# SpursLipu/YOLOv3v4-ModelCompression-MultidatasetTraining-Multibackbone

Measured on AMD Instinct MI355X. Metric: images/sec YOLOv3-608 train fp16, higher is better.
Workload: dtype f16; 1 GPU; YOLOv3 Darknet-53 608 COCO (80 classes) fp16 training step, batch 64/GPU: train-mode forward (batch-stat BN) + compute_loss + backward + nesterov SGD, single GPU; global_batch=64, parallelism=dp1

## Files before the change

yolov3v4-modelcompression-multidatasettraining-multibackbone_amd/csrc/conv_igemm.hip:

```cpp
#include "conv_igemm.h"

namespace yh {

template <typename T, int TM, int TN, int KU> struct MmaStep;

template <int TM, int TN, int KU> struct MmaStep<f16, TM, TN, KU> {
    static __device__ __forceinline__ void run(const u32x4* As, const u32x4* Bs, int BM, int BN, int arow, int brow,
                                               int lane, f32x4 (&acc)[TM][TN]) {
        const int r = lane & 15;
#pragma unroll
        for (int h = 0; h < KU / 4; ++h) {
            const int u = h * 4 + (lane >> 4);
            f16x8 a[TM], b[TN];
#pragma unroll
            for (int i = 0; i < TM; ++i) {
                u32x4 v = As[u * BM + arow + i * 16 + r];
                a[i] = *reinterpret_cast<f16x8*>(&v);
            }
#pragma unroll
            for (int j = 0; j < TN; ++j) {
                u32x4 v = Bs[u * BN + brow + j * 16 + r];
                b[j] = *reinterpret_cast<f16x8*>(&v);
            }
#pragma unroll
// ... 248 lines not shown
        for (int i = 0; i < TM; ++i)
#pragma unroll
            for (int j = 0; j < TN; ++j)
                acc[i][j] = __builtin_amdgcn_mfma_f32_16x16x32_f16(a[i], b[j], acc[i][j], 0, 0, 0);
    }
};
template <int TM, int TN> struct MmaStepRM<float, TM, TN> {
    static __device__ __forceinline__ void run(const u32x4* As, const u32x4* Bs, int arow, int brow, int lane,
                                               f32x4 (&acc)[TM][TN]) {
        const int r = lane & 15, kq = lane >> 4, fr = swz_f(r >> 2);
        const float* Af = reinterpret_cast<const float*>(As);
        const float* Bf = reinterpret_cast<const float*>(Bs);
#pragma unroll
        for (int u = 0; u < 4; ++u) {
            const int off = (r * 4 + (u ^ fr)) * 4 + kq;
            float a[TM], b[TN];
#pragma unroll
            for (int i = 0; i < TM; ++i) a[i] = Af[(arow + i * 16) * 16 + off];
#pragma unroll
            for (int j = 0; j < TN; ++j) b[j] = Bf[(brow + j * 16) * 16 + off];
#pragma unroll
            for (int i = 0; i < TM; ++i)
#pragma unroll
                for (int j = 0; j < TN; ++j)
                    acc[i][j] = __builtin_amdgcn_mfma_f32_16x16x4f32(a[i], b[j], acc[i][j], 0, 0, 0);
        }
    }
};

template <int TM, int TN> struct MmaStepRM<int8_t, TM, TN> {
    static __device__ __forceinline__ void run(const u32x4* As, const u32x4* Bs, int arow, int brow, int lane,
                                               i32x4 (&acc)[TM][TN]) {
        const int r = lane & 15;
        const int off = r * 4 + ((lane >> 4) ^ swz_f(r >> 2));
        i32x4 a[TM], b[TN];
#pragma unroll
        for (int i = 0; i < TM; ++i) {
            u32x4 v = As[(arow + i * 16) * 4 + off];
            a[i] = *reinterpret_cast<i32x4*>(&v);
        }
#pragma unroll
        for (int j = 0; j < TN; ++j) {
            u32x4 v = Bs[(brow + j * 16) * 4 + off];
            b[j] = *reinterpret_cast<i32x4*>(&v);
        }
#pragma unroll
        for (int i = 0; i < TM; ++i)
#pragma unroll
            for (int j = 0; j < TN; ++j)
                acc[i][j] = __builtin_amdgcn_mfma_i32_16x16x64_i8(a[i], b[j], acc[i][j], 0, 0, 0);
    }
};

template <typename T, typename OutT, int BM, int BN, int WM, int WN, int STAGES, int ABL = 0>
__global__ __launch_bounds__(WM * WN * 64, (WM * WN * 2) / 4) void conv_igemm_glds_kernel(const ConvArgs a) {
    constexpr int VEC = Prec<T>::VEC, BK = VEC * 4;
    constexpr int NW = WM * WN;
    constexpr int TM = BM / WM / 16, TN = BN / WN / 16;
    constexpr int GA = BM / 16, GB = BN / 16;
    constexpr int GPW = (GA + GB) / NW;
    constexpr int GAW = GA / NW;
    static_assert(GA % NW == 0 && GB % NW == 0, "tile rows must split evenly over the waves");
    static_assert(STAGES == 3 || STAGES == 4, "3 or 4 stage ring");

    __shared__ u32x4 smem[STAGES * 4 * (BM + BN)];
    constexpr int STAGE_CELLS = 4 * (BM + BN);

    const int lane = threadIdx.x & 63;
    const int wave = __builtin_amdgcn_readfirstlane(threadIdx.x >> 6);
    const int wm = wave / WN, wn = wave % WN;

    int m_tile, p_tile;
    {
        const int nb = gridDim.x, bid = blockIdx.x;
        const int q = nb >> 3, rr = nb & 7, xcd = bid & 7;
        const int logical = (xcd < rr ? xcd * (q + 1) : rr * (q + 1) + (xcd - rr) * q) + (bid >> 3);
        p_tile = logical / a.m_tiles;
        m_tile = logical - p_tile * a.m_tiles;
    }
    const int m0 = m_tile * BM;
    const long p0 = (long)p_tile * BN;

    const int lrow = lane >> 2;
    const int lu = (lane & 3) ^ swz_f(lane >> 4);
    const T* const xg = reinterpret_cast<const T*>(a.x);
    const T* const zero = reinterpret_cast<const T*>(g_zero_page);

    const T* wsrc[GAW > 0 ? GAW : 1];
    static_for<GAW>([&](auto c) {
        constexpr int i = decltype(c)::value;
        const int row = min(m0 + (wave + i * NW) * 16 + lrow, a.m_pad - 1);
        wsrc[i] = reinterpret_cast<const T*>(a.w) + (long)row * a.ktot + lu * VEC;
    });
    constexpr int GBW = GPW - GAW;
    long bbase[GBW];
    int bhi[GBW], bwi[GBW];
    const int HoWo = a.Ho * a.Wo;
    static_for<GBW>([&](auto c) {
        constexpr int i = decltype(c)::value;
        const int row = (wave + i * NW) * 16 + lrow;
        const long p = p0 + row;
        if (p < a.P) {
            const int n = (int)(p / HoWo);
            const int rem = (int)(p - (long)n * HoWo);
            const int ho = rem / a.Wo, wo = rem - ho * a.Wo;
            bhi[i] = ho * a.stride - a.pad;
            bwi[i] = wo * a.stride - a.pad;
            bbase[i] = (((long)n * a.H + bhi[i]) * a.W + bwi[i]) * a.ldx + lu * VEC;
        } else {
            bhi[i] = -(1 << 28);
            bwi[i] = -(1 << 28);
            bbase[i] = 0;
        }
    });

    int kr = 0, ks = 0, kc = 0, kofs = 0;
    auto issue = [&](int st) {
        u32x4* const base = smem + st * STAGE_CELLS;
        if constexpr (ABL != 1) static_for<GAW>([&](auto c) {
            constexpr int i = decltype(c)::value;
            u32x4* dst = base + (wave + i * NW) * 64;
            __builtin_amdgcn_global_load_lds((const __attribute__((address_space(1))) void*)(wsrc[i] + kofs),
                                             (__attribute__((address_space(3))) void*)dst, 16, 0, 0);
        });
        const long tap = ((long)kr * a.W + ks) * a.ldx + kc;
        const bool cok = kc + lu * VEC < a.Cin;
        if constexpr (ABL != 1) static_for<GBW>([&](auto c) {
            constexpr int i = decltype(c)::value;
            const bool ok = cok && (unsigned)(bhi[i] + kr) < (unsigned)a.H && (unsigned)(bwi[i] + ks) < (unsigned)a.W;
            const T* src = ok ? xg + bbase[i] + tap : zero;
            u32x4* dst = base + 4 * BM + (wave + i * NW) * 64;
            __builtin_amdgcn_global_load_lds((const __attribute__((address_space(1))) void*)src,
                                             (__attribute__((address_space(3))) void*)dst, 16, 0, 0);
        });
        kofs += BK;
        kc += BK;
        if (kc >= a.cin_k) {
            kc = 0;
            if (++ks == a.S) { ks = 0; ++kr; }
        }
    };

    typedef typename AccOf<T>::type acc_t;
    acc_t acc[TM][TN];
#pragma unroll
    for (int i = 0; i < TM; ++i)
#pragma unroll
        for (int j = 0; j < TN; ++j) acc[i][j] = acc_t{0, 0, 0, 0};

    const int nk = a.ktot / BK;
#pragma unroll
    for (int s = 0; s < STAGES - 1; ++s)
        if (s < nk) issue(s);
    int st_read = 0, st_write = STAGES - 1;
    for (int kt = 0; kt < nk; ++kt) {
        const int ahead = min(STAGES - 2, nk - 1 - kt);
        if (ahead >= 2) wait_vmcnt<2 * GPW>();
        else if (ahead == 1) wait_vmcnt<GPW>();
        else wait_vmcnt<0>();
        __builtin_amdgcn_s_barrier();
        if (kt + STAGES - 1 < nk) issue(st_write);
        const u32x4* As = smem + st_read * STAGE_CELLS;
        if constexpr (ABL != 2) MmaStepRM<T, TM, TN>::run(As, As + 4 * BM, wm * TM * 16, wn * TN * 16, lane, acc);
        st_read = st_read + 1 == STAGES ? 0 : st_read + 1;
        st_write = st_write + 1 == STAGES ? 0 : st_write + 1;
    }

    conv_epilogue<T, OutT, TM, TN, BN, WN>(a, acc, m0, p0, wm, wn, lane);
}

template <typename T, typename OutT, int BM, int BN, int WM, int WN, int STAGES, int ABL = 0>
static int launch_glds(const ConvArgs& a0, hipStream_t stream) {
    ConvArgs a = a0;
    a.m_tiles = (a.Cout + BM - 1) / BM;
    a.p_tiles = (int)((a.P + BN - 1) / BN);
    const long blocks = (long)a.m_tiles * a.p_tiles;
    if (blocks <= 0 || blocks > 0x7fffffffL) return YH_EINVAL;
    hipLaunchKernelGGL((conv_igemm_glds_kernel<T, OutT, BM, BN, WM, WN, STAGES, ABL>), dim3((unsigned)blocks),
                       dim3(WM * WN * 64), 0, stream, a);
    return check_launch();
}


template <typename T, typename OutT, int BM, int LB>
__global__ __launch_bounds__(512, (BM <= 128 ? 4 : 2)) void conv3x3_halo_kernel(const ConvArgs a, const int rows_h) {
    constexpr int VEC = Prec<T>::VEC, BK = VEC * 4, BN = 256, NW = 8, WN = 4, STAGES = 3;
    constexpr int WM = NW / WN;
    constexpr int TM = BM / WM / 16, TN = BN / WN / 16;
    constexpr int GAW = BM / 16 / NW;
    static_assert(BM % (16 * NW) == 0, "weight tile must split over 8 waves");
    constexpr int LA = GAW;

    extern __shared__ __attribute__((aligned(16))) u32x4 dsm[];
    u32x4* const Aring = dsm;
    u32x4* const Bbuf0 = dsm + STAGES * BM * 4;
    u32x4* const dummy = Bbuf0 + 2 * rows_h * 4;

    const int lane = threadIdx.x & 63;
    const int wave = __builtin_amdgcn_readfirstlane(threadIdx.x >> 6);
    const int wm = wave / WN, wn = wave % WN;

    int m_tile, p_tile;
    {
        const int nb = gridDim.x, bid = blockIdx.x;
        const int q = nb >> 3, rr = nb & 7, xcd = bid & 7;
        const int logical = (xcd < rr ? xcd * (q + 1) : rr * (q + 1) + (xcd - rr) * q) + (bid >> 3);
        p_tile = logical / a.m_tiles;
        m_tile = logical - p_tile * a.m_tiles;
    }
    const int m0 = m_tile * BM;
    const long q0 = (long)p_tile * BN;
    const int Wp = a.W + 2;
    const long IMG = (long)(a.H + 1) * Wp;

    const int lrow = lane >> 2;
    const int lu = (lane & 3) ^ (((lane >> 4) & 1) << 1);
    const T* const xg = reinterpret_cast<const T*>(a.x);
    const T* const zero = reinterpret_cast<const T*>(g_zero_page);

    const T* wsrc[GAW];
    static_for<GAW>([&](auto c) {
        constexpr int i = decltype(c)::value;
        const int row = min(m0 + (wave + i * NW) * 16 + lrow, a.m_pad - 1);
        wsrc[i] = reinterpret_cast<const T*>(a.w) + (long)row * a.ktot + lu * VEC;
    });
    const long v0 = q0 - Wp - 1;
    const T* bsrc[LB];
    static_for<LB>([&](auto c) {
        constexpr int i = decltype(c)::value;
        const int j = (wave + i * NW) * 16 + lrow;
        const long v = v0 + j;
// ... 363 lines not shown
    size_t lds;
    if (!yh::hpp_geometry(d->w_in, d->cin_k, bk, &rows_hp, &lb, &hbufs, &lds)) return false;
    if ((long)d->n * d->h * d->w_in * d->ldx + d->cin_k >= 0x7fffffffL || (long)d->m_pad * 9 * d->cin_k >= 0x7fffffffL) return false;
    const long blocks = (long)((d->cout + 127) / 128) * (((long)d->n * (d->h + 1) * (d->w_in + 1) + 511) / 512);
    const long rounds = (blocks + 255) / 256;
    return blocks >= 192 && (rounds >= 4 || blocks * 100 >= rounds * 256 * 60);
}

static bool pick_pointwise_tile(const yh_conv_desc* d) {
    static const bool off = getenv("YH_NO_POINTWISE") != nullptr;
    if (off || (d->dtype != YH_F16 && d->dtype != YH_I8)) return false;
    if (d->kh != 1 || d->kw != 1 || d->stride != 1 || d->pad != 0 || d->ups != 1 || d->res || d->stats_ws) return false;
    if (d->act != YH_ACT_LINEAR && d->act != YH_ACT_LEAKY && d->act != YH_ACT_MISH) return false;
    const int k = d->dtype == YH_I8 ? 64 : 32;
    if (d->cin != d->cin_k || d->cin_k % k || d->cout > 128) return false;
    const int mt = d->cout <= 32 ? 2 : (d->cout <= 64 ? 4 : 8), ks = d->cin_k / k;
    if (!((mt == 2 && (ks == 1 || ks == 2 || ks == 4)) || (mt == 4 && (ks == 1 || ks == 2)) || (mt == 8 && ks == 1))) return false;
    return (long)d->n * d->ho * d->wo >= 262144;
}

static bool stream3_supported(const yh_conv_desc* d) {
    if (d->dtype != YH_F16 && d->dtype != YH_I8) return false;
    if (d->kh != 3 || d->kw != 3 || d->pad != 1 || (d->stride != 1 && d->stride != 2) || d->ups != 1 || d->out_f32) return false;
    if (d->stats_ws && (d->dtype != YH_F16 || d->res)) return false;
    if (d->act != YH_ACT_LINEAR && d->act != YH_ACT_LEAKY && d->act != YH_ACT_MISH) return false;
    const bool two_steps = d->dtype == YH_F16 && d->cin_k == 64 && d->cout == 32 && !d->stats_ws;
    if (d->cin_k != (d->dtype == YH_I8 ? 64 : 32) && !two_steps) return false;
    if (d->cout != 32 && d->cout != 64 && !(d->cout == 128 && d->dtype == YH_I8)) return false;
    const int esz = d->dtype == YH_I8 ? 1 : 2;
    if ((d->ldy * esz) % 16 || (reinterpret_cast<uintptr_t>(d->y) & 15u)) return false;
    if ((long)d->n * d->ho * d->wo >= (1L << 31)) return false;
    return (long)d->n * d->h * d->w_in * d->ldx * esz < (1L << 31);
}
static bool pick_stream3_tile(const yh_conv_desc* d) {
    static const bool off = getenv("YH_NO_STREAM3") != nullptr;
    if (d->dtype == YH_F16 && d->cin_k != 32) return false;
    return !off && stream3_supported(d) && (long)d->n * d->ho * d->wo >= 262144;
}

static bool pwl_desc_supported(const yh_conv_desc* d) {
    if (d->kh != 1 || d->kw != 1 || d->stride != 1 || d->pad != 0 || d->ups != 1) return false;
    if (d->act != YH_ACT_LINEAR && d->act != YH_ACT_LEAKY && d->act != YH_ACT_MISH) return false;
    const bool bwd = d->bwd_z != nullptr;
    if (bwd && (d->act != YH_ACT_LINEAR || (d->bwd_act != YH_ACT_LEAKY && d->bwd_act != YH_ACT_MISH))) return false;
    return yh::pwl_supported(d->dtype, d->out_f32, d->cin, d->cin_k, d->cout, (long)d->n * d->ho * d->wo, d->ldx, d->ldy, d->ldr, d->x, d->y,
                             d->res, !bwd && d->stats_ws != nullptr, bwd);
}
static bool pick_pwl_tile(const yh_conv_desc* d) {
    static const bool off = getenv("YH_NO_PWL") != nullptr;
    static const long min_px = [] { const char* e = getenv("YH_PWL_MIN_PIXELS"); return e ? atol(e) : 262144L; }();
    return !off && pwl_desc_supported(d) && (long)d->n * d->ho * d->wo >= min_px;
}

extern "C" int yh_conv2d_tile(const yh_conv_desc* d) {
    if (!d) return YH_EINVAL;
    if (d->tile != 0) return d->tile;
    if (pick_pointwise_tile(d)) return 71;
    if (pick_pwl_tile(d)) return 73;
    if (pick_stream3_tile(d)) return 72;
    if (pick_hpp_tile(d)) return 43;
    if (pick_halo_tile(d)) return 41;
    if (const int pp = pick_pp_tile(d)) return pp;
    const int t = yh::pick_tile(d->cout, (long)d->n * d->ho * d->wo, d->cin_k, d->dtype == YH_F16 ? 8 : 4, d->kh * d->kw);
    if (d->ups == 2 && (t == 21 || t == 26 || t == 27 || t == 25)) {
        if (d->dtype == YH_F16) return 24;
        if (d->dtype == YH_I8) return 25;
    }
    if (d->dtype == YH_I8 && (t == 21 || t == 27) && (long)d->cin_k * d->kh * d->kw <= 256) return 25;
    return (d->dtype == YH_I8 && t == 3) ? 24 : t;
}

static bool tile_geometry(int tile, int* bn, int* wn) {
    switch (tile) {
        case 1: case 11: case 21: case 31: *bn = 128; *wn = 2; return true;
        case 2: case 12: case 22: case 32: case 3: *bn = 256; *wn = 4; return true;
        case 4: case 14: case 24: case 34: *bn = 128; *wn = 2; return true;
        case 5: case 15: case 25: case 35: *bn = 64; *wn = 2; return true;
        case 6: case 16: case 26: case 51: case 52: *bn = 128; *wn = 2; return true;
        case 27: case 61: case 64: case 67: *bn = 256; *wn = 4; return true;
        case 62: case 65: case 68: *bn = 512; *wn = 8; return true;
        case 63: case 66: case 69: *bn = 128; *wn = 2; return true;
        default: return false;
    }
}

extern "C" int64_t yh_conv2d_bwd_stats_rows(const yh_conv_desc* d) {
    if (!d || !d->bwd_z || !d->bwd_gamma || !d->bwd_beta || !d->bwd_mean || !d->bwd_invstd || d->n <= 0 || d->ho <= 0 || d->wo <= 0) return 0;
    if (d->dtype != YH_F16 || d->bwd_ldz % 8 || !yh::aligned16(d->bwd_z) || (d->tile != 0 && d->tile != 73)) return 0;
    static const bool off = getenv("YH_NO_BWD_SUMS") != nullptr;
    if (off || !pick_pwl_tile(d)) return 0;
    return (int64_t)yh::pwl_stats_rows((long)d->n * d->ho * d->wo, d->cout, true);
}

extern "C" int64_t yh_conv2d_stats_rows(const yh_conv_desc* d) {
    if (!d || d->n <= 0 || d->ho <= 0 || d->wo <= 0 || d->dtype == YH_I8) return 0;
    if (d->bwd_z) return 0;
    int bn, wn;
    yh_conv_desc q = *d;
    if (!q.stats_ws) q.stats_ws = reinterpret_cast<float*>(sizeof(float));
    const int tile = yh_conv2d_tile(&q);
    if (tile == 72) return (int64_t)yh::stream3_stats_rows((long)d->n * d->ho * d->wo, d->cout);
    if (tile == 73) return (int64_t)yh::pwl_stats_rows((long)d->n * d->ho * d->wo, d->cout);
    if (tile == 43)
        return (int64_t)(((long)d->n * (d->h + 1) * (d->w_in + 1) + 511) / 512) * 8;
    if (!tile_geometry(tile, &bn, &wn)) return 0;
    const long P = (long)d->n * d->ho * d->wo;
    return (int64_t)((P + bn - 1) / bn) * wn;
}

static void qadd_pow2_args(yh::ConvArgs& a) {
    const char* env = getenv("YH_QADD_POW2");
    if (env && env[0] == '0') return;
    int e[5];
    const float f[5] = {a.q_rx, a.q_ra, a.q_scale_x, a.q_scale_a, a.q_inv_scale_sum};
    for (int i = 0; i < 5; ++i) {
        int ex;
        if (!(f[i] > 0.f) || frexpf(f[i], &ex) != 0.5f) return;
        e[i] = ex - 1;
        if (e[i] < -40 || e[i] > 40) return;
    }
    if (e[0] < 0 || e[0] > 15 || e[1] < 0 || e[1] > 15) return;
    const int ex = e[0] + e[2], ea = e[1] + e[3];
    if (ex - ea > 15 || ea - ex > 15) return;
    a.q_rx = ldexpf(1.f, ex + e[4]);
    a.q_ra = ldexpf(1.f, ea + e[4]);
    a.q_scale_x = 0.f;
}

extern "C" int yh_conv2d_fwd(const yh_conv_desc* d, void* stream) {
    using namespace yh;
    if (!d || !d->x || !d->w || !d->bias || !d->y) return YH_EINVAL;
    if (d->n <= 0 || d->h <= 0 || d->w_in <= 0 || d->cin <= 0 || d->ho <= 0 || d->wo <= 0 || d->cout <= 0) return YH_EINVAL;
    if (d->kh <= 0 || d->kw <= 0 || d->stride <= 0 || d->pad < 0) return YH_EINVAL;
    if (d->dtype != YH_F16 && d->dtype != YH_F32 && d->dtype != YH_I8) return YH_EINVAL;
    const int bk = d->dtype == YH_F16 ? 32 : (d->dtype == YH_I8 ? 64 : 16), vec = d->dtype == YH_F16 ? 8 : (d->dtype == YH_I8 ? 16 : 4);
    if (d->dtype == YH_I8 && (!(d->acc_scale > 0.f) || !(d->out_scale > 0.f))) return YH_EINVAL;
    if (d->dtype == YH_I8 && d->res) {
        if (d->ups != 1 || d->out_f32 || !(d->q_rx > 0.f) || !(d->q_ra > 0.f) || !(d->q_scale_x > 0.f) || !(d->q_scale_a > 0.f) ||
            !(d->q_inv_scale_sum > 0.f) || d->ldr % 16 || (((uintptr_t)d->res) & 3u)) return YH_EINVAL;
        if (d->act != YH_ACT_LINEAR && d->act != YH_ACT_LEAKY && d->act != YH_ACT_MISH) return YH_EUNSUPPORTED;
    }
    if (d->cin % vec || d->ldx % vec || d->cin_k % bk || d->cin_k < d->cin || d->m_pad % 128 || d->m_pad < d->cout) return YH_EALIGN;
    if (d->cout % 4 || d->ldy % 4 || (d->res && d->ldr % 4)) return YH_EALIGN;
    if (!aligned16(d->x) || !aligned16(d->w) || !aligned16(d->bias) || (((uintptr_t)d->y) & 7u) || (((uintptr_t)d->res) & 7u)) return YH_EALIGN;
    if (d->ups < 1 || d->ups > 4) return YH_EINVAL;
    if (d->ups == 4) {
        if (d->dtype == YH_I8 || d->cout % 16 || d->cout < 64 || d->kh != 2 || d->kw != 2 || d->stride != 1 || d->pad != 0) return YH_EINVAL;
        if (d->tile != 0 && !(d->tile >= 21 && d->tile <= 35)) return YH_EINVAL;
        if (d->y_h <= 0 || d->y_w <= 0 || 2 * d->ho < d->y_h || 2 * d->wo < d->y_w || 2 * (d->ho - 1) >= d->y_h || 2 * (d->wo - 1) >= d->y_w) return YH_EINVAL;
        if (d->stats_ws) return YH_EINVAL;
    } else
    if (d->ups == 3) {
        if (d->dtype == YH_I8 || (d->tile >= 40 && d->tile < 50)) return YH_EINVAL;
        if (d->y_off_h < 0 || d->y_off_w < 0 || 2 * (d->ho - 1) + d->y_off_h >= d->y_h || 2 * (d->wo - 1) + d->y_off_w >= d->y_w) return YH_EINVAL;
    } else if (d->ho != (d->h + 2 * d->pad - d->kh) / d->stride + 1 || d->wo != (d->w_in + 2 * d->pad - d->kw) / d->stride + 1) {
        return YH_EINVAL;
    }

    ConvArgs a;
    a.x = d->x; a.w = d->w; a.bias = d->bias; a.res = d->res; a.y = d->y;
    a.N = d->n; a.H = d->h; a.W = d->w_in; a.Cin = d->cin; a.Ho = d->ho; a.Wo = d->wo; a.Cout = d->cout;
    a.R = d->kh; a.S = d->kw; a.stride = d->stride; a.pad = d->pad;
    a.ldx = d->ldx; a.ldr = d->ldr; a.ldy = d->ldy;
    a.cin_k = d->cin_k; a.ktot = d->kh * d->kw * d->cin_k;
    a.P = (long)d->n * d->ho * d->wo;
    a.m_tiles = a.p_tiles = 0;
    a.m_pad = d->m_pad;
    a.acc_scale = d->acc_scale; a.out_scale = d->out_scale; a.inv_out_scale = d->out_scale > 0.f ? 1.f / d->out_scale : 0.f;
    a.act = d->act; a.slope = d->slope; a.ups = d->ups;
    a.y_h = d->y_h; a.y_w = d->y_w; a.y_off_h = d->y_off_h; a.y_off_w = d->y_off_w;
    a.q_rx = d->q_rx; a.q_ra = d->q_ra; a.q_scale_x = d->q_scale_x; a.q_scale_a = d->q_scale_a; a.q_inv_scale_sum = d->q_inv_scale_sum;
    if (d->dtype == YH_I8 && d->res) qadd_pow2_args(a);
    a.no_lds_store = getenv("YH_PW_DIRECT") != nullptr;
    a.hpp_stagger = 0;
    a.stats_part = nullptr;
    a.bz = nullptr;
    a.bgamma = a.bbeta = a.bmean = a.binvstd = nullptr;
    a.ldbz = a.bact = 0;
    a.bslope = 0.f;
    if (d->bwd_z) {
        const int64_t rows = yh_conv2d_bwd_stats_rows(d);
        if (rows <= 0) return YH_EUNSUPPORTED;
        if (!d->stats_ws || d->stats_ws_floats < rows * 2 * d->cout) return YH_EINVAL;
        a.stats_part = d->stats_ws;
        a.bz = d->bwd_z; a.ldbz = d->bwd_ldz; a.bact = d->bwd_act; a.bslope = d->bwd_slope;
        a.bgamma = d->bwd_gamma; a.bbeta = d->bwd_beta; a.bmean = d->bwd_mean; a.binvstd = d->bwd_invstd;
        return launch_pwl_tile(a, d->dtype, (hipStream_t)stream);
    }
    if (d->stats_ws) {
        if (d->ups != 1 || d->res || d->dtype == YH_I8 || (d->tile >= 40 && d->tile < 50 && d->tile != 43)) return YH_EINVAL;
        const int64_t rows = yh_conv2d_stats_rows(d);
        if (rows <= 0 || d->stats_ws_floats < rows * 2 * d->cout) return YH_EINVAL;
        a.stats_part = d->stats_ws;
    }
    hipStream_t s = (hipStream_t)stream;
    int tile = d->tile;
    if (tile == 0) {
        tile = yh_conv2d_tile(d);
        if (d->ups == 4 && !(tile >= 21 && tile <= 35)) tile = 24;
    }
    if (tile == 71) {
        if (d->kh != 1 || d->kw != 1 || d->stride != 1 || d->pad != 0 || d->ups != 1 || d->res || d->stats_ws || d->cin != d->cin_k ||
            d->cout > 128 || d->dtype == YH_F32) return YH_EUNSUPPORTED;
        return launch_pointwise_tile(a, d->dtype, d->out_f32, s);
    }
    if (tile == 72) {
        if (!stream3_supported(d)) return YH_EUNSUPPORTED;
        return launch_stream3_tile(a, d->dtype, s);
    }
    if (tile == 73) {
        if (!pwl_desc_supported(d)) return YH_EUNSUPPORTED;
        return launch_pwl_tile(a, d->dtype, s);
    }
    if (d->dtype == YH_F16) {
        return d->out_f32 ? dispatch_tile<f16, float>(a, tile, s) : dispatch_tile<f16, f16>(a, tile, s);
    }
    if (d->dtype == YH_I8) {
        return d->out_f32 ? dispatch_tile_i8<float>(a, tile, s) : dispatch_tile_i8<int8_t>(a, tile, s);
    }
    return dispatch_tile<float, float>(a, tile, s);
}
```

yolov3v4-modelcompression-multidatasettraining-multibackbone_amd/engine/train.py:

```python
import ctypes as C
import os

import torch
import torch.nn as nn

from . import hiplib
from .hiplib import (ConvDesc, StemDesc, CopyDesc, AddDesc, BnStatsDesc, BnFinalizeDesc, BnActFwdDesc, BnBwdReduceDesc,
                     BnBwdApplyDesc, WgradDesc, StemWgradDesc, StemBwdDesc, UpsampleBwdDesc, CastDesc, LayoutDesc, PoolDesc, PoolBwdDesc, PackItem, PackBatchDesc, DwDesc, SeDesc, DwWgradDesc,
                     DwDgradDesc, SeBwdDesc, BnL1Row)
from .plan import DarknetEngine, ALIGN_C, _round_up

_FUSED_DGRAD_MAX_CIN = int(os.environ.get('YOLO_HIP_FUSED_DGRAD_MAX', '64'))

SLOT_INPUT = 0
SLOT_WS = 1
SLOT_WS2 = 63
SLOT_HEAD0 = 2
LINEAR = hiplib.ACT_CODES['linear']


class ChannelAlignmentError(NotImplementedError):
    """The aligned lowering wants every tensor width to be a multiple of 8: ``engine/padded.py`` trains such graphs through a
    channel-padded twin."""


class _Arena:

    def __init__(self):
        self.size = 0
        self.items = []

    def reserve(self, n):
        off = self.size
        self.size += _round_up(n, 4)
        return off

    def allocate(self, device):
        self.buf = torch.zeros(max(self.size, 4), device=device, dtype=torch.float32)
        return self.buf

    def ptr(self, off):
        return self.buf.data_ptr() + 4 * off

    def view(self, off, n):
        return self.buf[off:off + n]


class TrainEngine(DarknetEngine):
    def __init__(self, model, precision='fp16', lib=None):
        if precision not in ('fp16', 'fp32'):
            raise ValueError("training precision must be 'fp16' or 'fp32'")
        super().__init__(model, precision, lib)
        self._tplans = {}
        self._current = None
        self.steps = 0
        self._l1_blocks = ()
        self._l1_s = 0.0

    def parameters(self):
        out = []
        for block in self.model.module_list:
            if isinstance(block, nn.Sequential) and len(block) and isinstance(block[0], nn.Conv2d):
                conv, bn = block[0], None
                for k in list(block.children())[1:]:
                    if isinstance(k, nn.modules.batchnorm.BatchNorm2d):
                        bn = k
                out.append(conv.weight)
                if conv.bias is not None:
                    out.append(conv.bias)
                if bn is not None:
                    out.extend((bn.weight, bn.bias))
            elif isinstance(block, nn.Sequential) and len(block) and block[0].__class__.__name__ == 'SE':
                out.extend((block[0].fc[0].weight, block[0].fc[2].weight))
        return out

    def _pack_items(self, plan):
        items = []
        P = hiplib.ptr
        for v in plan['values']:
            if v.kind == 'dw':
                conv = v.conv
                for t in (conv.weight, conv.bias):
                    if t is not None and (t.dtype != torch.float32 or not t.is_contiguous()):
                        raise NotImplementedError('HIP training path: parameters must be contiguous fp32 (master weights)')
                items.append(PackItem(w=P(conv.weight), bias=P(conv.bias), packed=P(v.tpack['w']), bias_out=P(v.tpack['b']), mode=4,
                                      dtype=self.code, cout=v.C, cin=1, kh=v.k, kw=v.k, k_pad=v.c_phys, pad=v.pad))
                continue
            if v.kind != 'conv':
                continue
            conv, pk = v.conv, v.tpack
            for t in (conv.weight, conv.bias):
                if t is not None and (t.dtype != torch.float32 or not t.is_contiguous()):
                    raise NotImplementedError('HIP training path: parameters must be contiguous fp32 (master weights)')
            w, cb = P(conv.weight), P(conv.bias)
            geo = dict(dtype=self.code, cout=v.C, cin=conv.in_channels, kh=v.k, kw=v.k, pad=v.pad)
            if v.src.kind == 'input':
                items.append(PackItem(w=w, bias=cb, packed=P(pk['w']), bias_out=P(pk['b']), mode=3, cout_pad=pk['cout_pad'], **geo))
                continue
            items.append(PackItem(w=w, bias=cb, packed=P(pk['w']), bias_out=P(pk['b']), mode=0, k_pad=pk['cin_k'], m_pad=pk['m_pad'],
                                  **geo))
            if v.stride == 2 and pk.get('stem_fused'):
                items.append(PackItem(w=w, packed=P(pk['wt']), mode=1, k_pad=pk['cout_k'], m_pad=pk['dm_pad'], **geo))
            elif v.stride == 2 and 'wt_fused' in pk:
                items.append(PackItem(w=w, packed=P(pk['wt_fused']), mode=5, k_pad=pk['cout_k'], m_pad=pk['fused_m_pad'],
                                      cout_pad=v.src.c_phys, **geo))
            elif v.stride == 2:
                for (a, b), img in zip(((0, 0), (0, 1), (1, 0), (1, 1)), pk['wt_phase']):
                    items.append(PackItem(w=w, packed=P(img), mode=2, k_pad=pk['cout_k'], m_pad=pk['dm_pad'], pa=a, pb=b, **geo))
            else:
                items.append(PackItem(w=w, packed=P(pk['wt']), mode=1, k_pad=pk['cout_k'], m_pad=pk['dm_pad'], **geo))
        arr = (PackItem * len(items))(*items)
        return bytes(arr), len(items)

    def _refresh_pack_table(self, plan):
        ptrs = tuple(t.data_ptr() for t in self.parameters())
        if plan.get('pack_ptrs') == ptrs:
            return
        raw, n = self._pack_items(plan)
        host = torch.frombuffer(bytearray(raw), dtype=torch.uint8)
        if plan.get('pack_table') is None or plan['pack_table'].numel() != host.numel():
            raise RuntimeError('pack table size changed: rebuild the plan')
        plan['pack_table'].copy_(host)
        plan['pack_ptrs'] = ptrs

    def set_bn_sparsity(self, block_indices, s):
        blocks = tuple(sorted({int(b) for b in block_indices})) if block_indices is not None else ()
        if blocks:
            have = {}
            for i, block in enumerate(self.model.module_list):
                if isinstance(block, nn.Sequential) and len(block) and isinstance(block[0], nn.Conv2d):
                    have[i] = any(isinstance(k, nn.modules.batchnorm.BatchNorm2d) for k in list(block.children())[1:])
            bad = [b for b in blocks if not have.get(b, False)]
            if bad:
                raise ValueError('set_bn_sparsity: blocks %s are not conv blocks with BatchNorm' % bad)
        if blocks != self._l1_blocks:
            self._l1_blocks = blocks
            for plan in self._tplans.values():
                plan['l1_key'] = None
        self._l1_s = float(s) if blocks else 0.0

    def _l1_values(self, plan):
        want = set(self._l1_blocks)
        out = []
        for k, seg in enumerate(plan['segments']):
            lo, hi = seg['values']
            for v in plan['values'][lo:hi]:
                if v.kind in ('conv', 'dw') and v.bn is not None and v.block in want:
                    out.append((k, v))
        return out

    def _refresh_l1_table(self, plan):
        if not self._l1_blocks:
            plan['l1_key'], plan['l1_ranges'] = None, None
            return
# ... 127 lines not shown
                v.tpack = dict(w=torch.empty(v.k * v.k * v.c_phys, device=dev, dtype=self.dtype),
                               b=torch.empty(v.c_phys, device=dev, dtype=torch.float32))
                v.plain = bn is None and v.act == LINEAR
                v.z = None if v.plain else alloc((N, v.H, v.W, v.c_phys))
                v.res, v.ups, v.Ho, v.Wo, v.fp32 = None, 1, v.H, v.W, False
                continue
            if v.kind == 'se':
                v.p_first = len(plan['param_slices'])
                v.g_w1 = grads.reserve(v.fc1.weight.numel())
                plan['param_slices'].append((v.g_w1, v.fc1.weight.numel(), tuple(v.fc1.weight.shape)))
                v.g_w2 = grads.reserve(v.fc2.weight.numel())
                plan['param_slices'].append((v.g_w2, v.fc2.weight.numel(), tuple(v.fc2.weight.shape)))
                for t in (v.fc1.weight, v.fc2.weight):
                    if t.dtype != torch.float32 or not t.is_contiguous():
                        raise NotImplementedError('HIP training path: parameters must be contiguous fp32 (master weights)')
                v.pooled = alloc((N, v.c_phys), fp32=True)
                v.gate = alloc((N, v.c_phys), fp32=True)
                v.scratch = alloc((N, v.c_phys), fp32=True)
                v.scratch2 = alloc((N, v.c_phys + 2 * v.fc1.weight.shape[0]), fp32=True)
                continue
            if v.kind != 'conv':
                continue
            conv, bn = v.conv, v.bn
            taps = v.k * v.k
            v.p_first = len(plan['param_slices'])
            v.g_w = grads.reserve(conv.weight.numel())
            plan['param_slices'].append((v.g_w, conv.weight.numel(), tuple(conv.weight.shape)))
            v.g_b = None
            if conv.bias is not None:
                v.g_b = grads.reserve(v.c_phys)
                plan['param_slices'].append((v.g_b, v.C, (v.C,)))
            if bn is not None:
                v.g_gamma, v.g_beta = grads.reserve(v.C), grads.reserve(v.C)
                plan['param_slices'].append((v.g_gamma, v.C, (v.C,)))
                plan['param_slices'].append((v.g_beta, v.C, (v.C,)))
                v.s_sum, v.s_sumsq = stats.reserve(v.C), stats.reserve(v.C)
                v.s_mean, v.s_invstd = saved.reserve(v.C), saved.reserve(v.C)
            if v.src.kind == 'input':
                cout_pad = _round_up(v.C, 32) if v.C % 32 == 0 else _round_up(v.C, 16)
                v.tpack = dict(w=torch.empty(taps * v.src.C * cout_pad, device=dev, dtype=torch.float32),
                               b=torch.empty(cout_pad, device=dev, dtype=torch.float32), cout_pad=cout_pad)
            else:
                cin_k = _round_up(v.src.c_phys, kstep)
                m_pad = _round_up(v.c_phys, 128)
                cout_k = _round_up(v.c_phys, kstep)
                dm_pad = _round_up(v.src.c_phys, 128)
                v.tpack = dict(w=torch.empty(m_pad * taps * cin_k, device=dev, dtype=self.dtype),
                               b=torch.empty(m_pad, device=dev, dtype=torch.float32), cin_k=cin_k, m_pad=m_pad,
                               wt=None if v.stride == 2 else torch.empty(dm_pad * taps * cout_k, device=dev, dtype=self.dtype),
                               cout_k=cout_k, dm_pad=dm_pad)
                if self._dgrad_fused_into_stem(values, v):
                    v.tpack['stem_fused'] = True
                    v.tpack['wt'] = torch.empty(dm_pad * taps * cout_k, device=dev, dtype=self.dtype)
                elif v.stride == 2 and 16 <= v.src.c_phys <= _FUSED_DGRAD_MAX_CIN and v.src.c_phys % 4 == 0:
                    v.tpack['fused_m_pad'] = _round_up(4 * v.src.c_phys, 128)
                    v.tpack['wt_fused'] = torch.empty(v.tpack['fused_m_pad'] * 4 * cout_k, device=dev, dtype=self.dtype)
                elif v.stride == 2:
                    v.tpack['phase_taps'] = [((a + v.pad) // 2 + 1, (b + v.pad) // 2 + 1) for a in (0, 1) for b in (0, 1)]
                    v.tpack['wt_phase'] = [torch.empty(dm_pad * th * tw * cout_k, device=dev, dtype=self.dtype)
                                           for th, tw in v.tpack['phase_taps']]
            v.plain = bn is None and v.act == LINEAR and v.res is None and v.ups == 1
            if v.fp32:
                if not v.plain:
                    raise NotImplementedError('HIP training path: yolo-head conv with BN / activation / residual')
                v.z = None
            elif v.plain:
                v.z = None
            else:
                v.z = alloc((N, v.Ho, v.Wo, v.c_phys))
        plan['junk_n'] = max(v.c_phys for v in values if v.kind in ('conv', 'dw'))
        plan['junk'] = grads.reserve(plan['junk_n'])
        stats.allocate(dev)
        saved.allocate(dev)
        grads.allocate(dev)
        zero_bias = alloc((max([max(_round_up(v.src.c_phys, 128), v.tpack.get('fused_m_pad', 0))
                                for v in values if v.kind == 'conv' and v.src.kind != 'input'] + [128]),), fp32=True, zero=True)
        dz_elems = max(N * v.Ho * v.Wo * v.c_phys for v in values if v.kind in ('conv', 'dw'))
        lane_mode = int(os.environ.get('YOLO_HIP_WGRAD_LANE', '0') or 0)
        two_lanes = lane_mode > 0
        lane_ok = lambda u: lane_mode == 1 or (lane_mode == 2 and u.Ho <= 38) or (lane_mode == 3 and u.Ho <= 38 and u.k == 1)
        async_reduce = (not two_lanes and os.environ.get('YOLO_HIP_ASYNC_REDUCE', '0') == '1' and hasattr(lib, 'yh_plan_set_async_reduce'))
        dz_bufs = [alloc((dz_elems,)) for _ in range(2 if two_lanes else 1)]
        dz_state = dict(k=0, reader=[None] * len(dz_bufs))

        def next_dz():
            dz_state['k'] = (dz_state['k'] + 1) % len(dz_bufs)
            return dz_state['k']

        def dz_written_by(op, k):
            r = dz_state['reader'][k]
            if r is not None:
                hiplib.check(lib.yh_plan_add_dep(bwd, op, r), 'yh_plan_add_dep')
                dz_state['reader'][k] = None

        def on_side_lane(op, k):
            if not two_lanes:
                return
            hiplib.check(lib.yh_plan_set_lane(bwd, op, 1), 'yh_plan_set_lane')
            hiplib.check(lib.yh_plan_add_dep(bwd, op, op - 1), 'yh_plan_add_dep')
            dz_state['reader'][k] = op
        head_index = {id(h.src): k for k, h in enumerate(heads)}

        raw, n_items = self._pack_items(plan)
        plan['pack_table'] = torch.zeros(len(raw), device=dev, dtype=torch.uint8)
        plan['storages'].append(plan['pack_table'])
        add(fwd, plan['fwd_ops'], PackBatchDesc(items=plan['pack_table'].data_ptr(), n_items=n_items), 'pack')

        for v in values:
            if v.kind == 'input':
                continue
            y = None if v.storage is None else P(v.storage, v.c_off)
            if v.kind == 'conv':
                pk, s = v.tpack, v.src
                fused_stats = 0
                direct = v.plain
                zt = None if direct else v.z
                if s.kind == 'input':
                    d = StemDesc(x=None, w=P(pk['w']), bias=P(pk['b']), y=y if direct else P(zt), n=N, cin=s.C, h=s.H,
                                 w_in=s.W, ho=v.Ho, wo=v.Wo, cout=v.c_phys, cout_pad=pk['cout_pad'], kh=v.k, kw=v.k,
                                 stride=v.stride, pad=v.pad, ldy=v.ld if direct else v.c_phys, act=LINEAR, slope=0.0,
                                 dtype=self.code, out_scale=0.0)
                    if v.c_phys > pk['cout_pad'] or v.fp32:
                        raise NotImplementedError('HIP training path: stem geometry')
                    if v.bn is not None and not direct and os.environ.get('YOLO_HIP_STEM_STATS', '1') != '0':
                        fused_stats = int(lib.yh_conv2d_stem_stats_rows(C.byref(d)))
                        if fused_stats:
                            d.stats_ws_floats = fused_stats * 2 * v.c_phys
                            plan['ws_floats'] = max(plan['ws_floats'], d.stats_ws_floats)
# ... 282 lines not shown
                    if s.kind == 'input' and self._stem_bwd_fused(v, s):
                        sd = StemBwdDesc(x=None, dy=dyp, z=base['z'], gamma=bnp['gamma'], beta=bnp['beta'], mean=bnp['mean'],
                                         invstd=bnp['invstd'], dgamma=grads.ptr(v.g_gamma), dbeta=grads.ptr(v.g_beta),
                                         dw=grads.ptr(v.g_w), n=N, cin=s.C, h=s.H, w_in=s.W, cout=v.c_phys, lddy=lddy,
                                         ldz=v.c_phys, act=v.act, slope=v.slope)
                        for key, val in getattr(v, 'fused_dgrad', {}).items():
                            setattr(sd, key, val)
                        need = int(lib.yh_stem_bwd_workspace(C.byref(sd)))
                        if need <= 0:
                            raise RuntimeError('yh_stem_bwd_workspace rejected a geometry _stem_bwd_fused accepted')
                        sd.ws_floats = need
                        plan['ws_floats'] = max(plan['ws_floats'], need)
                        op = add(bwd, plan['bwd_ops'], sd, ('stembwd%d' if not getattr(v, 'fused_dgrad', None) else 'stembwd_dgrad%d') % v.block)
                        fixup(bwd, op, StemBwdDesc, 'ws', SLOT_WS)
                        fixup(bwd, op, StemBwdDesc, 'x', SLOT_INPUT)
                        continue
                    if not getattr(v, 'dbn_done', False):
                        add_reduction(bwd, plan['bwd_ops'], BnBwdReduceDesc(**base, **acc, dy=dyp, lddy=lddy), 'dbn%d' % v.block)
                    op = add(bwd, plan['bwd_ops'], BnBwdApplyDesc(**base, **acc, dy=dyp, lddy=lddy, out=dzp, ldo=v.c_phys),
                             'dbnx%d' % v.block)
                    dz_written_by(op, kz)
            if s.kind == 'input':
                img = alloc((N, s.H, s.W, ALIGN_C))
                op = add(bwd, plan['bwd_ops'], LayoutDesc(x=None, y=P(img), n=N, c=s.C, h=s.H, w_in=s.W, c_pad=ALIGN_C, ldy=ALIGN_C,
                                                          dtype=self.code), 'image%d' % v.block)
                fixup(bwd, op, LayoutDesc, 'x', SLOT_INPUT)
                side = two_lanes and dz_private and lane_ok(v)
                op = add_reduction(bwd, plan['bwd_ops'],
                                   WgradDesc(x=P(img), dz=dzp, dw=grads.ptr(v.g_w), n=N, h=s.H, w_in=s.W, cin=ALIGN_C, ho=v.Ho, wo=v.Wo,
                                             cout=v.C, kh=v.k, kw=v.k, stride=v.stride, pad=v.pad, ldx=ALIGN_C, lddz=lddz,
                                             dtype=self.code, splits=0, cin_w=s.C), 'wgrad%d' % v.block, side=side)
                if side:
                    on_side_lane(op, kz)
                continue
            side = two_lanes and dz_private and lane_ok(v)

            def emit_wgrad(v=v, s=s, dzp=dzp, lddz=lddz, kz=kz, side=side):
                op = add_reduction(bwd, plan['bwd_ops'],
                                   WgradDesc(x=P(s.storage, s.c_off), dz=dzp, dw=grads.ptr(v.g_w), n=N, h=s.H, w_in=s.W, cin=s.C, ho=v.Ho,
                                             wo=v.Wo, cout=v.C, kh=v.k, kw=v.k, stride=v.stride, pad=v.pad, ldx=s.ld, lddz=lddz,
                                             dtype=self.code, splits=0), 'wgrad%d' % v.block, side=side or async_reduce)
                if side:
                    on_side_lane(op, kz)
            if not side:
                emit_wgrad()
            mode = contribution_mode(s, True)
            common = dict(bias=P(zero_bias), n=N, cin=v.c_phys, cout=s.c_phys, stride=1, ldx=lddz, ldr=s.ld if mode == 'acc' else 0,
                          ldy=s.ld, cin_k=pk['cout_k'], m_pad=pk['dm_pad'], act=LINEAR, slope=0.0, out_f32=0, dtype=self.code,
                          tile=self.force_tile if self.force_tile < 40 else 0, acc_scale=0.0, out_scale=0.0)
            if pk.get('stem_fused'):
                if mode != 'write':
                    raise RuntimeError('fused first-block data gradient must be the only contribution to its gradient')
                s.fused_dgrad = dict(dz1=dzp, lddz1=lddz, w1=P(pk['wt']), h1=v.Ho, w1_in=v.Wo, k1=v.c_phys, k1_pad=pk['cout_k'])
            elif v.stride == 2 and 'wt_fused' in pk:
                fused = dict(common, cout=4 * s.c_phys, m_pad=pk['fused_m_pad'])
                if zero_bias.numel() < pk['fused_m_pad']:
                    raise RuntimeError('zero bias row is shorter than the fused data-gradient image')
                add(bwd, plan['bwd_ops'],
                    ConvDesc(x=dzp, w=P(pk['wt_fused']), res=gptr(s) if mode == 'acc' else None, y=gptr(s), h=v.Ho, w_in=v.Wo,
                             ho=(s.H + 1) // 2, wo=(s.W + 1) // 2, kh=2, kw=2, pad=0, ups=4, y_h=s.H, y_w=s.W, **fused),
                    'dgrad%d' % v.block)
            elif v.stride == 2:
                for (a, b), (th, tw), img in zip(((0, 0), (0, 1), (1, 0), (1, 1)), pk['phase_taps'], pk['wt_phase']):
                    hp, wp = (s.H - a + 1) // 2, (s.W - b + 1) // 2
                    if hp <= 0 or wp <= 0:
                        continue
                    add(bwd, plan['bwd_ops'],
                        ConvDesc(x=dzp, w=P(img), res=gptr(s) if mode == 'acc' else None, y=gptr(s), h=v.Ho, w_in=v.Wo, ho=hp, wo=wp,
                                 kh=th, kw=tw, pad=0, ups=3, y_h=s.H, y_w=s.W, y_off_h=a, y_off_w=b, **common),
                        'dgrad%d' % v.block)
            else:
                dg = ConvDesc(x=dzp, w=P(pk['wt']), res=gptr(s) if mode == 'acc' else None, y=gptr(s), h=v.Ho, w_in=v.Wo, ho=s.H,
                              wo=s.W, kh=v.k, kw=v.k, pad=v.k - 1 - v.pad, ups=1, **common)
                rows = 0
                if completes_bn_block(v, s):
                    sbase, sbnp = s.bn_args
                    for key, val in dict(bwd_z=sbase['z'], bwd_ldz=s.c_phys, bwd_act=s.act, bwd_slope=s.slope, bwd_gamma=sbnp['gamma'],
                                         bwd_beta=sbnp['beta'], bwd_mean=sbnp['mean'], bwd_invstd=sbnp['invstd']).items():
                        setattr(dg, key, val)
                    rows = int(lib.yh_conv2d_bwd_stats_rows(C.byref(dg)))
                    if rows <= 0:
                        for key in ('bwd_z', 'bwd_gamma', 'bwd_beta', 'bwd_mean', 'bwd_invstd'):
                            setattr(dg, key, None)
                if rows > 0:
                    dg.stats_ws_floats = rows * 2 * s.c_phys
                    plan['ws_floats'] = max(plan['ws_floats'], dg.stats_ws_floats)
                op = add(bwd, plan['bwd_ops'], dg, 'dgrad%d' % v.block)
                if rows > 0:
                    fixup(bwd, op, ConvDesc, 'stats_ws', SLOT_WS)
                    sacc = dict(sbnp, sum=grads.ptr(s.g_beta), sumsq=grads.ptr(s.g_gamma))
                    add_reduction(bwd, plan['bwd_ops'],
                                  BnBwdReduceDesc(**dict(sbase, ups=1), **sacc, dy=gptr(s), lddy=s.ld, nparts=rows), 'dbn%d' % s.block)
                    s.dbn_done = True
            if side:
                emit_wgrad()
        plan['head_shapes'] = [(N, h.src.H, h.src.W, h.src.c_phys) for h in heads]
        plan['segments'] = self._make_segments(plan, values, heads, bwd_pos)
        plan['ws'] = alloc((max(plan['ws_floats'], 4),), fp32=True)
        plan['ws2'] = alloc((max(plan['ws2_floats'], 4),), fp32=True)
        if async_reduce:
            hiplib.check(lib.yh_plan_set_async_reduce(bwd, 1), 'yh_plan_set_async_reduce')
        for handle in (fwd, bwd):
            lib.yh_plan_bind_slot(handle, SLOT_WS, plan['ws'].data_ptr())
        lib.yh_plan_bind_slot(bwd, SLOT_WS2, plan['ws2'].data_ptr())
        return plan

    def _stem_bwd_fused(self, v, s):
        if os.environ.get('YOLO_HIP_STEM_BWD', '1') == '0':
            return False
        return (self.code == hiplib.YH_F16 and v.bn is not None and v.k == 3 and v.stride == 1 and v.pad == 1 and s.C in (1, 3)
                and v.c_phys in (16, 32) and v.C == v.c_phys and v.ups == 1 and v.res is None and v.conv.bias is None)

    def _dgrad_fused_into_stem(self, values, v):
        s = v.src
        if os.environ.get('YOLO_HIP_STEM_DGRAD', '1') == '0' or os.environ.get('YOLO_HIP_WGRAD_LANE', '0') == '1':
            return False
        if v.kind != 'conv' or s.kind != 'conv' or s.src.kind != 'input' or not self._stem_bwd_fused(s, s.src):
            return False
        if not (v.k == 3 and v.stride == 2 and v.pad == 1 and v.C == 64 and v.c_phys == 64 and s.c_phys == 32 and not v.fp32):
            return False
        if s.parent is not None or s.c_off != 0 or s.ld != s.c_phys:
            return False
        users = 0
        for u in values:
            if u is v:
                continue
            refs = [getattr(u, 'src', None), getattr(u, 'res', None), getattr(u, 'a', None), getattr(u, 'b', None)]
            refs += [part[0] for part in getattr(u, 'parts', [])] if u.kind == 'concat' else []
            users += any(r is s for r in refs)
        return users == 0

    @staticmethod
    def _junk(plan, grads, n):
        junk = plan.get('junk')
        if junk is None or plan['junk_n'] < n:
            raise RuntimeError('junk accumulator was not reserved')
        return junk

    def _get_plan(self, x):
        if x.dim() != 4:
            raise ValueError('expected an (N, C, H, W) batch')
        if self.device is None:
            self.device = x.device
        elif self.device != x.device:
            raise RuntimeError('engine was built on %s, input is on %s' % (self.device, x.device))
        key = tuple(x.shape)
        plan = self._tplans.get(key)
        if plan is None:
            while len(self._tplans) >= 2:
                old = self._tplans.pop(next(iter(self._tplans)))
                for h in ('fwd', 'bwd'):
                    self.lib.yh_plan_destroy(old[h])
                if self._current is old:
                    self._current = None
            plan = self._tplans[key] = self._build_train_plan(*key)
        else:
            self._tplans[key] = self._tplans.pop(key)
        return plan

# ... 110 lines not shown
```

Before: 1222 images/s.

## Fuse four stride-2 dgrad phases into one all-phase implicit-GEMM launch

```diff
diff --git a/yolov3v4-modelcompression-multidatasettraining-multibackbone_amd/csrc/conv_igemm.hip b/yolov3v4-modelcompression-multidatasettraining-multibackbone_amd/csrc/conv_igemm.hip
--- a/yolov3v4-modelcompression-multidatasettraining-multibackbone_amd/csrc/conv_igemm.hip
+++ b/yolov3v4-modelcompression-multidatasettraining-multibackbone_amd/csrc/conv_igemm.hip
@@ -324,7 +324,7 @@
     }
 };
 
-template <typename T, typename OutT, int BM, int BN, int WM, int WN, int STAGES, int ABL = 0>
+template <typename T, typename OutT, int BM, int BN, int WM, int WN, int STAGES, int ABL = 0, bool ALLPH = false>
 __global__ __launch_bounds__(WM * WN * 64, (WM * WN * 2) / 4) void conv_igemm_glds_kernel(const ConvArgs a) {
     constexpr int VEC = Prec<T>::VEC, BK = VEC * 4;
     constexpr int NW = WM * WN;
@@ -352,6 +352,9 @@
     }
     const int m0 = m_tile * BM;
     const long p0 = (long)p_tile * BN;
+    const int ph = ALLPH ? m0 / (a.Cout >> 2) : 0;
+    const int pa = ph >> 1, pb = ph & 1;
+    const int wrow0 = ALLPH ? m0 - ph * (a.Cout >> 2) : m0;
 
     const int lrow = lane >> 2;
     const int lu = (lane & 3) ^ swz_f(lane >> 4);
@@ -361,7 +364,7 @@
     const T* wsrc[GAW > 0 ? GAW : 1];
     static_for<GAW>([&](auto c) {
         constexpr int i = decltype(c)::value;
-        const int row = min(m0 + (wave + i * NW) * 16 + lrow, a.m_pad - 1);
+        const int row = min(wrow0 + (wave + i * NW) * 16 + lrow, a.m_pad - 1);
         wsrc[i] = reinterpret_cast<const T*>(a.w) + (long)row * a.ktot + lu * VEC;
     });
     constexpr int GBW = GPW - GAW;
@@ -389,6 +392,7 @@
     int kr = 0, ks = 0, kc = 0, kofs = 0;
     auto issue = [&](int st) {
         u32x4* const base = smem + st * STAGE_CELLS;
+        if constexpr (ALLPH) kofs = ((pa ? 2 * kr : 1) * 3 + (pb ? 2 * ks : 1)) * a.cin_k + kc;
         if constexpr (ABL != 1) static_for<GAW>([&](auto c) {
             constexpr int i = decltype(c)::value;
             u32x4* dst = base + (wave + i * NW) * 64;
@@ -409,7 +413,7 @@
         kc += BK;
         if (kc >= a.cin_k) {
             kc = 0;
-            if (++ks == a.S) { ks = 0; ++kr; }
+            if (++ks == (ALLPH ? pb + 1 : a.S)) { ks = 0; ++kr; }
         }
     };
 
@@ -420,7 +424,7 @@
 #pragma unroll
         for (int j = 0; j < TN; ++j) acc[i][j] = acc_t{0, 0, 0, 0};
 
-    const int nk = a.ktot / BK;
+    const int nk = ALLPH ? (pa + 1) * (pb + 1) * (a.cin_k / BK) : a.ktot / BK;
 #pragma unroll
     for (int s = 0; s < STAGES - 1; ++s)
         if (s < nk) issue(s);
@@ -441,14 +445,15 @@
     conv_epilogue<T, OutT, TM, TN, BN, WN>(a, acc, m0, p0, wm, wn, lane);
 }
 
-template <typename T, typename OutT, int BM, int BN, int WM, int WN, int STAGES, int ABL = 0>
+template <typename T, typename OutT, int BM, int BN, int WM, int WN, int STAGES, int ABL = 0, bool ALLPH = false>
 static int launch_glds(const ConvArgs& a0, hipStream_t stream) {
     ConvArgs a = a0;
+    if (ALLPH && (a.ups != 4 || (a.Cout & 3) || (a.Cout >> 2) % BM)) return YH_EUNSUPPORTED;
     a.m_tiles = (a.Cout + BM - 1) / BM;
     a.p_tiles = (int)((a.P + BN - 1) / BN);
     const long blocks = (long)a.m_tiles * a.p_tiles;
     if (blocks <= 0 || blocks > 0x7fffffffL) return YH_EINVAL;
-    hipLaunchKernelGGL((conv_igemm_glds_kernel<T, OutT, BM, BN, WM, WN, STAGES, ABL>), dim3((unsigned)blocks),
+    hipLaunchKernelGGL((conv_igemm_glds_kernel<T, OutT, BM, BN, WM, WN, STAGES, ABL, ALLPH>), dim3((unsigned)blocks),
                        dim3(WM * WN * 64), 0, stream, a);
     return check_launch();
 }
@@ -918,8 +923,24 @@
     return !off && pwl_desc_supported(d) && (long)d->n * d->ho * d->wo >= min_px;
 }
 
+static int allphase_tile(const yh_conv_desc* d) {
+    if (d->dtype != YH_F16 || d->out_f32 || d->stats_ws || d->bwd_z || d->act != YH_ACT_LINEAR) return YH_EUNSUPPORTED;
+    if (d->kh != 3 || d->kw != 3 || d->stride != 2 || d->pad != 1 || d->cout % 64 || d->cin_k % 32) return YH_EUNSUPPORTED;
+    if (d->y_h <= 0 || d->y_w <= 0 || d->ho != (d->y_h + 1) / 2 || d->wo != (d->y_w + 1) / 2 || d->h != d->ho || d->w_in != d->wo) return YH_EUNSUPPORTED;
+    const bool wide = d->cout % 128 == 0;
+    if (d->tile != 0) {
+        if (wide ? (d->tile != 21 && d->tile != 27) : (d->tile != 22 && d->tile != 24)) return YH_EUNSUPPORTED;
+        return d->tile;
+    }
+    const long P = (long)d->n * d->ho * d->wo;
+    const long wide_blocks = (long)(4 * d->cout / 128) * ((P + 255) / 256);
+    if (wide) return wide_blocks >= 512 ? 27 : 21;
+    return (long)(4 * d->cout / 64) * ((P + 255) / 256) >= 512 ? 22 : 24;
+}
+
 extern "C" int yh_conv2d_tile(const yh_conv_desc* d) {
     if (!d) return YH_EINVAL;
+    if (d->ups == 5) return allphase_tile(d);
     if (d->tile != 0) return d->tile;
     if (pick_pointwise_tile(d)) return 71;
     if (pick_pwl_tile(d)) return 73;
@@ -1009,7 +1030,10 @@
     if (d->cin % vec || d->ldx % vec || d->cin_k % bk || d->cin_k < d->cin || d->m_pad % 128 || d->m_pad < d->cout) return YH_EALIGN;
     if (d->cout % 4 || d->ldy % 4 || (d->res && d->ldr % 4)) return YH_EALIGN;
     if (!aligned16(d->x) || !aligned16(d->w) || !aligned16(d->bias) || (((uintptr_t)d->y) & 7u) || (((uintptr_t)d->res) & 7u)) return YH_EALIGN;
-    if (d->ups < 1 || d->ups > 4) return YH_EINVAL;
+    if (d->ups < 1 || d->ups > 5) return YH_EINVAL;
+    if (d->ups == 5) {
+        if (allphase_tile(d) < 0) return YH_EUNSUPPORTED;
+    } else
     if (d->ups == 4) {
         if (d->dtype == YH_I8 || d->cout % 16 || d->cout < 64 || d->kh != 2 || d->kw != 2 || d->stride != 1 || d->pad != 0) return YH_EINVAL;
         if (d->tile != 0 && !(d->tile >= 21 && d->tile <= 35)) return YH_EINVAL;
@@ -1044,6 +1068,17 @@
     a.bgamma = a.bbeta = a.bmean = a.binvstd = nullptr;
     a.ldbz = a.bact = 0;
     a.bslope = 0.f;
+    if (d->ups == 5) {
+        a.Cout = 4 * d->cout; a.R = a.S = 2; a.stride = 1; a.pad = 0; a.ups = 4;
+        hipStream_t s5 = (hipStream_t)stream;
+        switch (allphase_tile(d)) {
+            case 27: return launch_glds<f16, f16, 128, 256, 2, 4, 3, 0, true>(a, s5);
+            case 21: return launch_glds<f16, f16, 128, 128, 2, 2, 3, 0, true>(a, s5);
+            case 22: return launch_glds<f16, f16, 64, 256, 1, 4, 3, 0, true>(a, s5);
+            case 24: return launch_glds<f16, f16, 64, 128, 2, 2, 3, 0, true>(a, s5);
+            default: return YH_EUNSUPPORTED;
+        }
+    }
     if (d->bwd_z) {
         const int64_t rows = yh_conv2d_bwd_stats_rows(d);
         if (rows <= 0) return YH_EUNSUPPORTED;
diff --git a/yolov3v4-modelcompression-multidatasettraining-multibackbone_amd/engine/train.py b/yolov3v4-modelcompression-multidatasettraining-multibackbone_amd/engine/train.py
--- a/yolov3v4-modelcompression-multidatasettraining-multibackbone_amd/engine/train.py
+++ b/yolov3v4-modelcompression-multidatasettraining-multibackbone_amd/engine/train.py
@@ -11,6 +11,7 @@
 from .plan import DarknetEngine, ALIGN_C, _round_up
 
 _FUSED_DGRAD_MAX_CIN = int(os.environ.get('YOLO_HIP_FUSED_DGRAD_MAX', '64'))
+_ALLPHASE_DGRAD_MIN_CIN = int(os.environ.get('YOLO_HIP_ALLPHASE_DGRAD_MIN', '128'))
 
 SLOT_INPUT = 0
 SLOT_WS = 1
@@ -99,7 +100,7 @@
                 continue
             items.append(PackItem(w=w, bias=cb, packed=P(pk['w']), bias_out=P(pk['b']), mode=0, k_pad=pk['cin_k'], m_pad=pk['m_pad'],
                                   **geo))
-            if v.stride == 2 and pk.get('stem_fused'):
+            if v.stride == 2 and (pk.get('stem_fused') or 'allphase_rows' in pk):
                 items.append(PackItem(w=w, packed=P(pk['wt']), mode=1, k_pad=pk['cout_k'], m_pad=pk['dm_pad'], **geo))
             elif v.stride == 2 and 'wt_fused' in pk:
                 items.append(PackItem(w=w, packed=P(pk['wt_fused']), mode=5, k_pad=pk['cout_k'], m_pad=pk['fused_m_pad'],
@@ -333,6 +334,9 @@
                 if self._dgrad_fused_into_stem(values, v):
                     v.tpack['stem_fused'] = True
                     v.tpack['wt'] = torch.empty(dm_pad * taps * cout_k, device=dev, dtype=self.dtype)
+                elif v.stride == 2 and self._dgrad_allphase(v, N, cout_k, dm_pad):
+                    v.tpack['allphase_rows'] = 4 * v.src.c_phys
+                    v.tpack['wt'] = torch.empty(dm_pad * taps * cout_k, device=dev, dtype=self.dtype)
                 elif v.stride == 2 and 16 <= v.src.c_phys <= _FUSED_DGRAD_MAX_CIN and v.src.c_phys % 4 == 0:
                     v.tpack['fused_m_pad'] = _round_up(4 * v.src.c_phys, 128)
                     v.tpack['wt_fused'] = torch.empty(v.tpack['fused_m_pad'] * 4 * cout_k, device=dev, dtype=self.dtype)
@@ -354,7 +358,7 @@
         stats.allocate(dev)
         saved.allocate(dev)
         grads.allocate(dev)
-        zero_bias = alloc((max([max(_round_up(v.src.c_phys, 128), v.tpack.get('fused_m_pad', 0))
+        zero_bias = alloc((max([max(_round_up(v.src.c_phys, 128), v.tpack.get('fused_m_pad', 0), v.tpack.get('allphase_rows', 0))
                                 for v in values if v.kind == 'conv' and v.src.kind != 'input'] + [128]),), fp32=True, zero=True)
         dz_elems = max(N * v.Ho * v.Wo * v.c_phys for v in values if v.kind in ('conv', 'dw'))
         lane_mode = int(os.environ.get('YOLO_HIP_WGRAD_LANE', '0') or 0)
@@ -743,6 +747,13 @@
                 if mode != 'write':
                     raise RuntimeError('fused first-block data gradient must be the only contribution to its gradient')
                 s.fused_dgrad = dict(dz1=dzp, lddz1=lddz, w1=P(pk['wt']), h1=v.Ho, w1_in=v.Wo, k1=v.c_phys, k1_pad=pk['cout_k'])
+            elif v.stride == 2 and 'allphase_rows' in pk:
+                if zero_bias.numel() < pk['allphase_rows']:
+                    raise RuntimeError('zero bias row is shorter than the all-phase data gradient reads')
+                add(bwd, plan['bwd_ops'],
+                    ConvDesc(x=dzp, w=P(pk['wt']), res=gptr(s) if mode == 'acc' else None, y=gptr(s), h=v.Ho, w_in=v.Wo,
+                             ho=(s.H + 1) // 2, wo=(s.W + 1) // 2, kh=3, kw=3, pad=1, ups=5, y_h=s.H, y_w=s.W, **dict(common, stride=2)),
+                    'dgrad%d' % v.block)
             elif v.stride == 2 and 'wt_fused' in pk:
                 fused = dict(common, cout=4 * s.c_phys, m_pad=pk['fused_m_pad'])
                 if zero_bias.numel() < pk['fused_m_pad']:
@@ -796,6 +807,16 @@
         lib.yh_plan_bind_slot(bwd, SLOT_WS2, plan['ws2'].data_ptr())
         return plan
 
+    def _dgrad_allphase(self, v, N, cout_k, dm_pad):
+        s, tile_of = v.src, getattr(self.lib, 'yh_conv2d_tile', None)
+        if (tile_of is None or self.code != hiplib.YH_F16 or _ALLPHASE_DGRAD_MIN_CIN <= 0 or s.c_phys < _ALLPHASE_DGRAD_MIN_CIN
+                or v.k != 3 or v.stride != 2 or v.pad != 1):
+            return False
+        d = ConvDesc(n=N, h=v.Ho, w_in=v.Wo, cin=v.c_phys, ho=(s.H + 1) // 2, wo=(s.W + 1) // 2, cout=s.c_phys, kh=3, kw=3, stride=2, pad=1,
+                     ldx=v.c_phys, ldy=s.ld, cin_k=cout_k, m_pad=dm_pad, act=LINEAR, slope=0.0, ups=5, out_f32=0, dtype=self.code,
+                     tile=self.force_tile if self.force_tile < 40 else 0, y_h=s.H, y_w=s.W)
+        return int(tile_of(C.byref(d))) > 0
+
     def _stem_bwd_fused(self, v, s):
         if os.environ.get('YOLO_HIP_STEM_BWD', '1') == '0':
             return False
```

Measured after the change: 1222 images/s. Within noise of the previous version (-0.0%).
